# tatsy/opengl-raytracer

Measured on AMD Instinct MI355X. Metric: Mrays/s at 1920x1080, 8 bounces, higher is better.
Workload: dtype f32

## Files before the change

opengl-raytracer_amd/csrc/glrtx.hip:

```cpp
#include "glrtx.h"

#include <hip/hip_runtime.h>

#include <algorithm>
#include <cmath>
#include <cstdarg>
#include <cstdio>
#include <cstdlib>
#include <cstring>
#include <new>
#include <limits>
#include <string>
#include <vector>

#include "glrt_host.h"
#include "pt_kernel.hip.h"
#include "accumulate.hip.h"
#include "lbvh.hip.h"
#include "sahl.hip.h"
#include "refit.hip.h"
#include "skin.hip.h"
#include "normals.hip.h"
#include "query.hip.h"
#include "features.hip.h"
// ... 4253 lines not shown
    nt = std::min(nt, lg.cap_trips);
    std::vector<uint2> tr(nt);
    HIP_TRY(c, hipMemcpy(tr.data(), lg.trips, (size_t)nt * sizeof(uint2), hipMemcpyDeviceToHost));
    unsigned long long logged = 0;
    for (const uint2 &t : tr) logged += t.y;
    DbgLastLaunch L = g_dbg_last;
    L.w.suspend_max = 0;
    using RKernel = void (*)(const KernelArgs, const WfArgs, unsigned *, float4 *, const float4 *, const uint2 *, int);
    int fetch = L.fetch;
    if (const char *v = std::getenv("GLRTX_REPLAY_PAIR_FETCH")) fetch = std::max(0, std::min(2, std::atoi(v)));
    const RKernel rk = fetch == 2 ? (RKernel)pt_replay_traverse<2> : fetch == 1 ? (RKernel)pt_replay_traverse<1> : (RKernel)pt_replay_traverse<0>;
    if (L.lds > 64 * 1024) HIP_TRY(c, hipFuncSetAttribute((const void *)rk, hipFuncAttributeMaxDynamicSharedMemorySize, L.lds));
    int per_cu = 0;
    HIP_TRY(c, hipOccupancyMaxActiveBlocksPerMultiprocessor(&per_cu, rk, kBlockThreads, L.lds));
    if (const char *v = std::getenv("GLRTX_WGS_PER_CU")) per_cu = std::max(1, std::min(per_cu, std::atoi(v)));
    const int grid = std::max(1, std::min(L.grid, per_cu * c->n_cu));
    float ms = 0.f;
    for (int r = 0; r < reps; r++) {
        HIP_TRY(c, hipMemsetAsync(c->work.p, 0, sizeof(unsigned), c->stream));
        HIP_TRY(c, hipEventRecord(c->tm0, c->stream));
        hipLaunchKernelGGL(rk, dim3(grid), dim3(kBlockThreads), L.lds, c->stream, L.a, L.w, (unsigned *)c->work.p, L.queues,
                           (const float4 *)lg.rays, (const uint2 *)lg.trips, (int)nt);
        HIP_TRY(c, hipGetLastError());
        HIP_TRY(c, hipEventRecord(c->tm1, c->stream));
        HIP_TRY(c, hipEventSynchronize(c->tm1));
        HIP_TRY(c, hipEventElapsedTime(&ms, c->tm0, c->tm1));
    }
    out[0] = ms; out[1] = (double)logged; out[2] = (double)nt; out[3] = (double)n;
    return GLRTX_OK;
}
#endif

#ifdef GLRTX_STEP_TIMING
int glrtx_debug_step_timing(unsigned long long out[4]) { return take_symbol(g_step_timing, out); }
#endif

#ifdef GLRTX_PHASE_STATS
int glrtx_debug_trip_log(unsigned out[16 * 64 * 4]) { return take_symbol(g_trip_log, out); }
int glrtx_debug_phase_cycles(unsigned long long out[8]) { return take_symbol(g_phase_cycles, out); }
#endif

int glrtx_timer_begin(glrtx_ctx *c) {
    if (!c) return GLRTX_EINVAL;
    seal_feed(c);
    HIP_TRY(c, hipSetDevice(c->device));
    HIP_TRY(c, hipEventRecord(c->tm0, c->stream));
    return GLRTX_OK;
}

int glrtx_timer_end(glrtx_ctx *c, float *ms) {
    if (!c || !ms) return GLRTX_EINVAL;
    seal_feed(c);
    HIP_TRY(c, hipSetDevice(c->device));
    HIP_TRY(c, hipEventRecord(c->tm1, c->stream));
    HIP_TRY(c, hipEventSynchronize(c->tm1));
    HIP_TRY(c, hipEventElapsedTime(ms, c->tm0, c->tm1));
    return GLRTX_OK;
}

}

struct glrtx_group {
    std::vector<glrtx_ctx *> ctx;
    std::vector<hipEvent_t> done;
    DevBuf full, full8;
    std::vector<char> peer_ok;
    int gather_copies = 0;
// ... 374 lines not shown
```

opengl-raytracer_amd/csrc/pt_kernel.hip.h:

```cpp
#pragma once
#include <hip/hip_runtime.h>
#include <stdint.h>

#include "trav_asm.hip.h"
#include "scan_asm.hip.h"

namespace glrtx {

constexpr int kBlockThreads = 256;
constexpr int kTile = 16;
constexpr int REF_ABSENT = INT32_MIN;
constexpr int REF_FIN = INT32_MIN;
constexpr int kMaxLdsMaterials = 256;
constexpr int kMaxLdsLights = 64;
constexpr int kTopForks = 128;

constexpr float PT_EPS = 1.0e-4f;
constexpr float PT_INFTY = 1.0e8f;
constexpr float PT_PI = 3.14159274101257324f;
constexpr float PT_2PI = 6.28318548202514648f;

struct DevScene {
    const float4 *forks;
    const float4 *nodes0;
// ... 374 lines not shown
        unsigned addr;
        const unsigned lds_base = (unsigned)(uintptr_t)stack;
        asm volatile(
            "s_mov_b64 %[save], exec\n"
            "1:\n\t"
            "v_cmp_ne_u32 vcc, 0, %[sp]\n\t"
            "v_cndmask_b32 %[ref], %[fin], %[ref], vcc\n\t"
            "s_and_b64 exec, exec, vcc\n\t"
            "s_cbranch_execz 2f\n\t"
            "v_add_u32 %[sp], -1, %[sp]\n\t"
            "v_lshl_add_u32 %[addr], %[sp], 11, %[base]\n\t"
            "ds_read_b32 %[ref], %[addr] offset:4\n\t"
            "ds_read_b32 %[t0], %[addr]\n\t"
            "s_waitcnt lgkmcnt(0)\n\t"
            "v_cmp_gt_f32 vcc, %[t0], %[th]\n\t"
            "s_and_b64 exec, exec, vcc\n\t"
            "s_cbranch_execnz 1b\n"
            "2:\n\t"
            "s_mov_b64 exec, %[save]"
            : [t0] "=&v"(t0), [ref] "+&v"(ref), [sp] "+&v"(sp), [save] "=&s"(save), [addr] "=&v"(addr)
            : [base] "v"(lds_base), [th] "v"(T.h.t), [fin] "v"(REF_FIN)
            : "vcc", "scc", "memory");
        static_assert(kBlockThreads * 8 == 1 << 11, "the pop loop shifts the stack index by 11: entry e of lane l at byte (e * kBlockThreads + l) * 8");
        T.sp = sp;
        T.cur = ref;
    }
#ifdef GLRTX_TRAV_STATS
    if (T.cur == REF_FIN) { TS_DONE; }
#endif
    return T.cur == REF_FIN;
}

#ifdef GLRTX_STEP_TIMING
__device__ unsigned long long g_step_timing[4];
struct StepTiming { unsigned t = 0, w = 0, n = 0; };
#define GLRTX_TS_PARAM , StepTiming &ST
#define GLRTX_TS_OPERANDS , [tt] "+&v"(ST.t), [tw] "+&v"(ST.w), [tn] "+&v"(ST.n)
#define GLRTX_TS_CLOBBERS , "s90", "s91", "s92", "s93", "s94", "s95"
#else
#define GLRTX_TS_PARAM
#define GLRTX_TS_OPERANDS
#define GLRTX_TS_CLOBBERS
#endif
constexpr int kWgwfCompact = 8;
constexpr int kWgwfVolume = 16;
template <int FETCH>
DEV void trav_steps_asm(const DevScene &sc, int *stack, Trav &T, unsigned rk GLRTX_TS_PARAM) {
    unsigned long long s_entry, s_act, s_leaf, s_bl, s_br, s_pop, s_tmp;
    const unsigned stk = (unsigned)(uintptr_t)stack;
    static_assert(kBlockThreads * 8 == 1 << 11, "trav_asm.hip.h shifts the stack index by 11: entry e of lane l at byte (e * kBlockThreads + l) * 8");
    static_assert(REF_FIN == INT32_MIN, "trav_asm.hip.h materialises REF_FIN with v_bfrev_b32 v, 1");
    const unsigned par16 = (threadIdx.x & 1u) << 4;
    const unsigned bias_e = sc.node_bias + par16, bias_o = sc.node_bias + 16u - par16;
    if constexpr ((FETCH & kWgwfCompact) != 0) {
        static_assert((FETCH & ~kWgwfCompact) == 0, "the compact layout has the one-record-per-lane fetch only");
        asm volatile(
            "s_mov_b64 %[entry], exec\n\t"
            "s_mov_b64 %[act], exec\n\t"
            GLRTX_ASM_SET_VBASE
            "v_bfrev_b32 v[GLRTX_VB+22], 1\n\t"
            GLRTX_REP(GLRTX_STEPS_PER_TRIP, GLRTX_TRAV_STEP_ASM_COMPACT)
            "99:\n\t"
            "s_mov_b64 exec, %[entry]"
            : [th] "+&v"(T.h.t), [tri] "+&v"(T.h.tri), [hu] "+&v"(T.h.u), [hv] "+&v"(T.h.v), [cur] "+&v"(T.cur), [sp] "+&v"(T.sp),
              [entry] "=&s"(s_entry), [act] "=&s"(s_act), [leaf] "=&s"(s_leaf), [bl] "=&s"(s_bl), [br] "=&s"(s_br), [pop] "=&s"(s_pop), [tmp] "=&s"(s_tmp) GLRTX_TS_OPERANDS
            : [ox] "v"(T.ox), [oy] "v"(T.oy), [oz] "v"(T.oz), [dx] "v"(T.dx), [dy] "v"(T.dy), [dz] "v"(T.dz), [ix] "v"(T.ix), [iy] "v"(T.iy), [iz] "v"(T.iz),
              [sd] "v"(T.stop_d), [stk] "v"(stk), [cbase] "s"(sc.cnodes), [rk] "s"(rk), [eps] "s"(PT_EPS)
            : "vcc", "scc", "memory", GLRTX_ASM_VCLOBBERS_COMPACT GLRTX_TS_CLOBBERS);
        return;
    }
    if (FETCH == 2) {
        asm volatile(
            "s_mov_b64 %[entry], exec\n\t"
            "s_mov_b64 %[act], exec\n\t"
            GLRTX_ASM_SET_VBASE
            "v_bfrev_b32 v[GLRTX_VB+11], 1\n\t"
            GLRTX_REP(GLRTX_STEPS_PER_TRIP_HALF, GLRTX_TRAV_STEP_ASM_PAIR GLRTX_TRAV_STEP_ASM_LANE)
            "99:\n\t"
            "s_mov_b64 exec, %[entry]"
            : [th] "+&v"(T.h.t), [tri] "+&v"(T.h.tri), [hu] "+&v"(T.h.u), [hv] "+&v"(T.h.v), [cur] "+&v"(T.cur), [sp] "+&v"(T.sp),
              [entry] "=&s"(s_entry), [act] "=&s"(s_act), [leaf] "=&s"(s_leaf), [bl] "=&s"(s_bl), [br] "=&s"(s_br), [pop] "=&s"(s_pop), [tmp] "=&s"(s_tmp) GLRTX_TS_OPERANDS
            : [ox] "v"(T.ox), [oy] "v"(T.oy), [oz] "v"(T.oz), [dx] "v"(T.dx), [dy] "v"(T.dy), [dz] "v"(T.dz), [ix] "v"(T.ix), [iy] "v"(T.iy), [iz] "v"(T.iz),
              [sd] "v"(T.stop_d), [stk] "v"(stk), [base] "s"(sc.nodes0), [bias] "s"(sc.node_bias), [eps] "s"(PT_EPS),
              [odd] "s"(0xAAAAAAAAAAAAAAAAull), [biase] "v"(bias_e), [biaso] "v"(bias_o)
            : "vcc", "scc", "memory", GLRTX_ASM_VCLOBBERS_PAIR GLRTX_TS_CLOBBERS);
        return;
    }
    if (FETCH == 1) {
        asm volatile(
            "s_mov_b64 %[entry], exec\n\t"
            "s_mov_b64 %[act], exec\n\t"
            GLRTX_ASM_SET_VBASE
            "v_bfrev_b32 v[GLRTX_VB+11], 1\n\t"
            GLRTX_REP(GLRTX_STEPS_PER_TRIP, GLRTX_TRAV_STEP_ASM_PAIR)
            "99:\n\t"
            "s_mov_b64 exec, %[entry]"
            : [th] "+&v"(T.h.t), [tri] "+&v"(T.h.tri), [hu] "+&v"(T.h.u), [hv] "+&v"(T.h.v), [cur] "+&v"(T.cur), [sp] "+&v"(T.sp),
              [entry] "=&s"(s_entry), [act] "=&s"(s_act), [leaf] "=&s"(s_leaf), [bl] "=&s"(s_bl), [br] "=&s"(s_br), [pop] "=&s"(s_pop), [tmp] "=&s"(s_tmp) GLRTX_TS_OPERANDS
            : [ox] "v"(T.ox), [oy] "v"(T.oy), [oz] "v"(T.oz), [dx] "v"(T.dx), [dy] "v"(T.dy), [dz] "v"(T.dz), [ix] "v"(T.ix), [iy] "v"(T.iy), [iz] "v"(T.iz),
              [sd] "v"(T.stop_d), [stk] "v"(stk), [base] "s"(sc.nodes0), [eps] "s"(PT_EPS),
              [odd] "s"(0xAAAAAAAAAAAAAAAAull), [biase] "v"(bias_e), [biaso] "v"(bias_o)
            : "vcc", "scc", "memory", GLRTX_ASM_VCLOBBERS_PAIR GLRTX_TS_CLOBBERS);
        return;
    }
    asm volatile(
        "s_mov_b64 %[entry], exec\n\t"
        "s_mov_b64 %[act], exec\n\t"
        GLRTX_ASM_SET_VBASE
        "v_bfrev_b32 v[GLRTX_VB+11], 1\n\t"
        GLRTX_REP(GLRTX_STEPS_PER_TRIP, GLRTX_TRAV_STEP_ASM_LANE)
        "99:\n\t"
        "s_mov_b64 exec, %[entry]"
        : [th] "+&v"(T.h.t), [tri] "+&v"(T.h.tri), [hu] "+&v"(T.h.u), [hv] "+&v"(T.h.v), [cur] "+&v"(T.cur), [sp] "+&v"(T.sp),
          [entry] "=&s"(s_entry), [act] "=&s"(s_act), [leaf] "=&s"(s_leaf), [bl] "=&s"(s_bl), [br] "=&s"(s_br), [pop] "=&s"(s_pop), [tmp] "=&s"(s_tmp) GLRTX_TS_OPERANDS
        : [ox] "v"(T.ox), [oy] "v"(T.oy), [oz] "v"(T.oz), [dx] "v"(T.dx), [dy] "v"(T.dy), [dz] "v"(T.dz), [ix] "v"(T.ix), [iy] "v"(T.iy), [iz] "v"(T.iz),
          [sd] "v"(T.stop_d), [stk] "v"(stk), [base] "s"(sc.nodes0), [bias] "s"(sc.node_bias), [eps] "s"(PT_EPS)
        : "vcc", "scc", "memory", GLRTX_ASM_VCLOBBERS GLRTX_TS_CLOBBERS);
}

template <bool CLOSEST>
DEV void tri_test(Hit &h, int t, float ox, float oy, float oz, float dx, float dy, float dz, float v0x, float v0y, float v0z, float e1x,
                  float e1y, float e1z, float e2x, float e2y, float e2z, float tmin = PT_EPS) {
    const float tx = ox - v0x, ty = oy - v0y, tz = oz - v0z;
    const float px = dy * e2z - dz * e2y;
    const float py = dz * e2x - dx * e2z;
    const float pz = dx * e2y - dy * e2x;
    const float det = dot3(e1x, e1y, e1z, px, py, pz);
    const float U = dot3(tx, ty, tz, px, py, pz);
    const float inv = rcp_newton(det);
    const float u = U * inv;
    const bool ok_u = !(-PT_EPS < det && det < PT_EPS) && !(u < 0.0f || 1.0f < u);
    if (!__any(ok_u)) return;
    const float qx = ty * e1z - tz * e1y;
    const float qy = tz * e1x - tx * e1z;
    const float qz = tx * e1y - ty * e1x;
    const float V = dot3(dx, dy, dz, qx, qy, qz);
    const float v = V * inv;
    const bool ok_v = ok_u && !(v < 0.0f || 1.0f < inv * (U + V));
    if (!__any(ok_v)) return;
    const float tt = dot3(e2x, e2y, e2z, qx, qy, qz) * inv;
    const bool hit = ok_v && !(tmin >= tt);
    const bool closer = hit && tt < h.t;
    h.tri = closer ? t : h.tri;
    if (CLOSEST) { h.u = closer ? u : h.u; h.v = closer ? v : h.v; }
// ... 1408 lines not shown
#endif
        if (active) {
#if defined(GLRTX_TRAV_STATS) || defined(GLRTX_CXX_STEP)
            constexpr bool CP = (FETCH & kWgwfCompact) != 0;
            bool fin = trav_step<true, CP>(a.sc, stack, T, ranks);
#pragma unroll
            for (int k = 1; k < GLRTX_STEPS_PER_TRIP; k++)
                if (!fin) fin = trav_step<true, CP>(a.sc, stack, T, ranks);
#else
#ifdef GLRTX_STEP_TIMING
            trav_steps_asm<FETCH>(a.sc, stack, T, (unsigned)(uintptr_t)ranks, step_timing);
#else
            trav_steps_asm<FETCH>(a.sc, stack, T, (unsigned)(uintptr_t)ranks);
#endif
            const bool fin = T.cur == REF_FIN;
#endif
            if (fin) {
                active = false;
                unsaved = true;
            }
        }
#ifdef GLRTX_PHASE_STATS
        ph_step += __builtin_amdgcn_s_memtime() - sb0;
#endif
    }
    if (unsaved) save_hit();
#ifdef GLRTX_PHASE_STATS
    if (threadIdx.x == 0) { atomicAdd(&g_phase_cycles[5], ph_refill); atomicAdd(&g_phase_cycles[6], ph_refills); atomicAdd(&g_phase_cycles[7], ph_step); }
#endif
#ifdef GLRTX_STEP_TIMING
    atomicAdd(&g_step_timing[0], (unsigned long long)step_timing.n);
    atomicAdd(&g_step_timing[1], (unsigned long long)step_timing.t);
    atomicAdd(&g_step_timing[2], (unsigned long long)step_timing.w);
#endif
}

template <bool VOL = false>
DEV void wg_shade_phase(const KernelArgs &a, const WfArgs &w, const float4 *lds_mats, const float *cam, const unsigned *light_bits, int n_paths,
                        float4 *rq_next, unsigned *n_rays_next, unsigned *n_paths_next, unsigned cur_base, unsigned next_base, unsigned long long &rays,
                        unsigned *moved) {
    const int lane = threadIdx.x & 63;
    const unsigned long long lt_mask = (1ull << lane) - 1ull;
    for (int j0 = 0; j0 < n_paths; j0 += kBlockThreads) {
        const int i = j0 + (int)threadIdx.x;
        bool push_ext = false, push_sh = false, requeue = false, has4 = false;
        unsigned id = WF_INVALID;
        float4 ro = make_float4(0.f, 0.f, 0.f, 0.f), rd = ro, rsd = ro, st2 = ro, st3 = ro, st4 = ro;
        const bool light_accepted = i < n_paths && ((light_bits[i >> 5] >> (i & 31)) & 1u) != 0u;
        if (i < n_paths)
            wf_shade_path<VOL>(a, w, lds_mats, cam, id, cur_base + (unsigned)i, light_accepted, push_ext, push_sh, requeue, ro, rd, rsd, st2, st3, st4, has4, rays);
        const unsigned long long me = __ballot(push_ext), ms = __ballot(push_sh), mq = __ballot(requeue), mp = me | ms | mq;
        const unsigned long long mv = __ballot(id != WF_INVALID);
        unsigned br = 0, bp = 0;
        if (lane == 0) {
            if (mv & ~mq) *moved = 1u;
            if (mp) {
                br = atomicAdd(n_rays_next, (unsigned)(__popcll(me) + __popcll(ms)));
                bp = atomicAdd(n_paths_next, (unsigned)__popcll(mp));
            }
        }
        br = __builtin_amdgcn_readfirstlane(br);
        bp = __builtin_amdgcn_readfirstlane(bp);
        const unsigned pos_next = bp + (unsigned)__popcll(mp & lt_mask);
        const unsigned sidx_next = next_base + pos_next;
        if (push_ext || push_sh || requeue) {
            st_stream(w.A(0, sidx_next), ro);
// ... 503 lines not shown
```

opengl-raytracer_amd/csrc/trav_asm.hip.h:

```cpp
#pragma once

#ifndef GLRTX_STEPS_PER_TRIP
#define GLRTX_STEPS_PER_TRIP 6
#endif
#ifndef GLRTX_ASM_VBASE
#define GLRTX_ASM_VBASE 96
#endif
static_assert(GLRTX_STEPS_PER_TRIP % 2 == 0, "the alternating form of the node fetch unrolls steps in pairs");
#define GLRTX_STEPS_PER_TRIP_HALF_(n) GLRTX_HALF_##n
#define GLRTX_HALF_2 1
#define GLRTX_HALF_4 2
#define GLRTX_HALF_6 3
#define GLRTX_HALF_8 4
#define GLRTX_STEPS_PER_TRIP_HALF_X(n) GLRTX_STEPS_PER_TRIP_HALF_(n)
#define GLRTX_STEPS_PER_TRIP_HALF GLRTX_STEPS_PER_TRIP_HALF_X(GLRTX_STEPS_PER_TRIP)
#define GLRTX_STR_(x) #x
#define GLRTX_STR(x) GLRTX_STR_(x)
#define GLRTX_ASM_SET_VBASE ".set GLRTX_VB, " GLRTX_STR(GLRTX_ASM_VBASE) "\n\t"
#if GLRTX_ASM_VBASE == 96
#define GLRTX_ASM_VCLOBBERS "v96", "v97", "v98", "v99", "v100", "v101", "v102", "v103", "v104", "v105", "v106", "v107", "v108", "v109", "v110", "v111", "v112", "v113", "v114", "v115", "v116", "v117"
#define GLRTX_ASM_VCLOBBERS_PAIR GLRTX_ASM_VCLOBBERS, "v118", "v119"
#define GLRTX_ASM_VCLOBBERS_COMPACT GLRTX_ASM_VCLOBBERS_PAIR
#elif GLRTX_ASM_VBASE == 72
#define GLRTX_ASM_VCLOBBERS "v72", "v73", "v74", "v75", "v76", "v77", "v78", "v79", "v80", "v81", "v82", "v83", "v84", "v85", "v86", "v87", "v88", "v89", "v90", "v91", "v92", "v93"
#define GLRTX_ASM_VCLOBBERS_PAIR GLRTX_ASM_VCLOBBERS, "v94", "v95"
#define GLRTX_ASM_VCLOBBERS_COMPACT GLRTX_ASM_VCLOBBERS_PAIR
#else
#error "GLRTX_ASM_VBASE: add the clobber list for this base"
#endif

#ifdef GLRTX_STEP_TIMING
#define GLRTX_TS_BEGIN "s_memtime s[90:91]\n\t"
#define GLRTX_TS_WAIT0 "s_memtime s[92:93]\n\t"
#define GLRTX_TS_WAIT1 "s_memtime s[94:95]\n\ts_waitcnt lgkmcnt(0)\n\ts_sub_u32 s92, s94, s92\n\t"
#define GLRTX_TS_END "s_memtime s[94:95]\n\ts_waitcnt lgkmcnt(0)\n\ts_sub_u32 s94, s94, s90\n\tv_add_u32 %[tt], s94, %[tt]\n\tv_add_u32 %[tw], s92, %[tw]\n\tv_add_u32 %[tn], 1, %[tn]\n\t"
#else
#define GLRTX_TS_BEGIN
#define GLRTX_TS_WAIT0
#define GLRTX_TS_WAIT1
#define GLRTX_TS_END
#endif


#if defined(GLRTX_STEP_TIMING)
#define GLRTX_SINGLE_WAIT
#endif
#ifndef GLRTX_SINGLE_WAIT
#define GLRTX_W3 "s_waitcnt vmcnt(3)\n\t"
#define GLRTX_W2 "s_waitcnt vmcnt(2)\n\t"
#define GLRTX_W1 "s_waitcnt vmcnt(1)\n\t"
#define GLRTX_W0 "s_waitcnt vmcnt(0)\n\t"
#else
#define GLRTX_W3 "s_waitcnt vmcnt(0)\n\t"
#define GLRTX_W2
#define GLRTX_W1
#define GLRTX_W0
#endif
#define GLRTX_TRAV_STEP_ASM_PAIR \
    GLRTX_TS_BEGIN \
    "s_andn2_b64 %[tmp], %[act], %[odd]\n\t"    \
    "s_lshl_b64 %[tmp], %[tmp], 1\n\t" \
    "s_and_b64 %[pop], %[act], %[odd]\n\t" \
    "s_lshr_b64 %[pop], %[pop], 1\n\t" \
    "s_or_b64 %[tmp], %[tmp], %[pop]\n\t" \
    "s_or_b64 %[pop], %[tmp], %[act]\n\t"    \
    "s_mov_b64 exec, %[pop]\n\t" \
    "v_cndmask_b32_e64 v[GLRTX_VB+4], -1, %[cur], %[act]\n\t"    \
    "v_cmp_gt_i32_e64 %[leaf], 0, %[cur]\n\t"    \
    "s_nop 0\n\t"    \
    "v_mov_b32_dpp v[GLRTX_VB+15], v[GLRTX_VB+4] quad_perm:[0,0,2,2] row_mask:0xf bank_mask:0xf\n\t"    \
    "v_mov_b32_dpp v[GLRTX_VB+23], v[GLRTX_VB+4] quad_perm:[1,1,3,3] row_mask:0xf bank_mask:0xf\n\t"    \
    "v_lshl_add_u32 v[GLRTX_VB+15], v[GLRTX_VB+15], 6, %[biase]\n\t"    \
// ... 176 lines not shown
    "v_max_f32 v[GLRTX_VB+17], v[GLRTX_VB+5], v[GLRTX_VB+1]\n\t" \
    "v_min_f32 v[GLRTX_VB+1], v[GLRTX_VB+5], v[GLRTX_VB+1]\n\t" \
    "v_max_f32 v[GLRTX_VB+18], v[GLRTX_VB+6], v[GLRTX_VB+2]\n\t" \
    "v_min_f32 v[GLRTX_VB+4], v[GLRTX_VB+6], v[GLRTX_VB+2]\n\t" \
    "v_min3_f32 v[GLRTX_VB+16], v[GLRTX_VB+16], v[GLRTX_VB+17], v[GLRTX_VB+18]\n\t"    \
    "v_max3_f32 v[GLRTX_VB+2], v[GLRTX_VB+0], v[GLRTX_VB+1], v[GLRTX_VB+4]\n\t"        \
    "v_min_f32 v[GLRTX_VB+16], v[GLRTX_VB+16], %[th]\n\t" \
    "v_cmp_ge_f32_e64 %[bl], v[GLRTX_VB+16], v[GLRTX_VB+2]\n\t"                      \
    GLRTX_CW0 \
    "v_sub_f32 v[GLRTX_VB+8], v[GLRTX_VB+8], %[ox]\n\t"    \
    "v_sub_f32 v[GLRTX_VB+9], v[GLRTX_VB+9], %[oy]\n\t" \
    "v_sub_f32 v[GLRTX_VB+10], v[GLRTX_VB+10], %[oz]\n\t" \
    "v_mul_f32 v[GLRTX_VB+8], v[GLRTX_VB+8], %[ix]\n\t" \
    "v_mul_f32 v[GLRTX_VB+9], v[GLRTX_VB+9], %[iy]\n\t" \
    "v_mul_f32 v[GLRTX_VB+10], v[GLRTX_VB+10], %[iz]\n\t" \
    "v_sub_f32 v[GLRTX_VB+12], v[GLRTX_VB+3], %[ox]\n\t" \
    "v_sub_f32 v[GLRTX_VB+13], v[GLRTX_VB+7], %[oy]\n\t" \
    "v_sub_f32 v[GLRTX_VB+14], v[GLRTX_VB+11], %[oz]\n\t" \
    "v_mul_f32 v[GLRTX_VB+12], v[GLRTX_VB+12], %[ix]\n\t" \
    "v_mul_f32 v[GLRTX_VB+13], v[GLRTX_VB+13], %[iy]\n\t" \
    "v_mul_f32 v[GLRTX_VB+14], v[GLRTX_VB+14], %[iz]\n\t" \
    "v_max_f32 v[GLRTX_VB+16], v[GLRTX_VB+12], v[GLRTX_VB+8]\n\t" \
    "v_min_f32 v[GLRTX_VB+8], v[GLRTX_VB+12], v[GLRTX_VB+8]\n\t" \
    "v_max_f32 v[GLRTX_VB+17], v[GLRTX_VB+13], v[GLRTX_VB+9]\n\t" \
    "v_min_f32 v[GLRTX_VB+9], v[GLRTX_VB+13], v[GLRTX_VB+9]\n\t" \
    "v_max_f32 v[GLRTX_VB+18], v[GLRTX_VB+14], v[GLRTX_VB+10]\n\t" \
    "v_min_f32 v[GLRTX_VB+10], v[GLRTX_VB+14], v[GLRTX_VB+10]\n\t" \
    "v_min3_f32 v[GLRTX_VB+16], v[GLRTX_VB+16], v[GLRTX_VB+17], v[GLRTX_VB+18]\n\t" \
    "v_max3_f32 v[GLRTX_VB+8], v[GLRTX_VB+8], v[GLRTX_VB+9], v[GLRTX_VB+10]\n\t" \
    "v_min_f32 v[GLRTX_VB+16], v[GLRTX_VB+16], %[th]\n\t" \
    "v_cmp_ge_f32_e64 %[br], v[GLRTX_VB+16], v[GLRTX_VB+8]\n\t" \
    "v_lshl_add_u32 v[GLRTX_VB+3], v[GLRTX_VB+19], 1, 1\n\t"                         \
    "v_add_u32 v[GLRTX_VB+7], 1, v[GLRTX_VB+3]\n\t"                                  \
    GLRTX_TRAV_STEP_TAIL_X("", "v[GLRTX_VB+22]")
#define GLRTX_TRAV_STEP_TAIL GLRTX_TRAV_STEP_TAIL_X("v_not_b32 v[GLRTX_VB+3], %[cur]\n\t", "v[GLRTX_VB+11]")
#define GLRTX_TRAV_STEP_TAIL_X(TRI, FIN) \
    "v_cndmask_b32_e64 %[cur], v[GLRTX_VB+3], v[GLRTX_VB+7], %[br]\n\t"                                  \
    "s_or_b64 %[tmp], %[bl], %[br]\n\t"                                                                                                                \
    "s_andn2_b64 %[pop], exec, %[tmp]\n\t"                                                                     \
    "s_and_b64 exec, %[bl], %[br]\n\t"                                                               \
    "v_lshl_add_u32 v[GLRTX_VB+15], %[sp], 11, %[stk]\n\t"                                                                                                       \
    "ds_write_b64 v[GLRTX_VB+15], v[GLRTX_VB+2:GLRTX_VB+3]\n\t"                                                                                                                  \
    "v_add_u32 %[sp], 1, %[sp]\n\t"                                                                                                                    \
    "s_and_b64 exec, %[act], %[leaf]\n\t"                                \
    "s_cbranch_scc0 21f\n\t"                                                                                                                           \
    TRI                                                                                                                                      \
    "v_mov_b32 %[cur], v[GLRTX_VB+7]\n\t"                                                   \
    "v_mul_f32 v[GLRTX_VB+16], %[dy], v[GLRTX_VB+10]\n\t"                                                                                                  \
    "v_mul_f32 v[GLRTX_VB+19], %[dz], v[GLRTX_VB+9]\n\t"                                                                                                                  \
    "v_sub_f32 v[GLRTX_VB+16], v[GLRTX_VB+16], v[GLRTX_VB+19]\n\t"                                                                                                                   \
    "v_mul_f32 v[GLRTX_VB+17], %[dz], v[GLRTX_VB+8]\n\t"                                                                                                                  \
    "v_mul_f32 v[GLRTX_VB+19], %[dx], v[GLRTX_VB+10]\n\t"                                                                                                                  \
    "v_sub_f32 v[GLRTX_VB+17], v[GLRTX_VB+17], v[GLRTX_VB+19]\n\t"                                                                                                                   \
    "v_mul_f32 v[GLRTX_VB+18], %[dx], v[GLRTX_VB+9]\n\t"                                                                                                                  \
    "v_mul_f32 v[GLRTX_VB+19], %[dy], v[GLRTX_VB+8]\n\t"                                                                                                                  \
    "v_sub_f32 v[GLRTX_VB+18], v[GLRTX_VB+18], v[GLRTX_VB+19]\n\t"                                                                                                                   \
    "v_mul_f32 v[GLRTX_VB+20], v[GLRTX_VB+6], v[GLRTX_VB+18]\n\t"                                                                          \
    "v_mul_f32 v[GLRTX_VB+19], v[GLRTX_VB+5], v[GLRTX_VB+17]\n\t"                                                                                                                   \
    "v_add_f32 v[GLRTX_VB+20], v[GLRTX_VB+20], v[GLRTX_VB+19]\n\t"                                                                                                                   \
    "v_mul_f32 v[GLRTX_VB+19], v[GLRTX_VB+4], v[GLRTX_VB+16]\n\t"                                                                                                                   \
    "v_add_f32 v[GLRTX_VB+20], v[GLRTX_VB+20], v[GLRTX_VB+19]\n\t"                                                                                                                   \
    "v_rcp_f32 v[GLRTX_VB+21], v[GLRTX_VB+20]\n\t"                                                                                                                         \
    "v_sub_f32 v[GLRTX_VB+0], %[ox], v[GLRTX_VB+0]\n\t"                                                                                          \
    "v_sub_f32 v[GLRTX_VB+1], %[oy], v[GLRTX_VB+1]\n\t"                                                                                                                    \
    "v_sub_f32 v[GLRTX_VB+2], %[oz], v[GLRTX_VB+2]\n\t"                                                                                                                    \
    "v_fma_f32 v[GLRTX_VB+19], -v[GLRTX_VB+20], v[GLRTX_VB+21], 1.0\n\t"                                                           \
    "v_fma_f32 v[GLRTX_VB+21], v[GLRTX_VB+19], v[GLRTX_VB+21], v[GLRTX_VB+21]\n\t"                                                                                                             \
    "v_mul_f32 v[GLRTX_VB+18], v[GLRTX_VB+2], v[GLRTX_VB+18]\n\t"                                                                                   \
    "v_mul_f32 v[GLRTX_VB+19], v[GLRTX_VB+1], v[GLRTX_VB+17]\n\t"                                                                                                                    \
    "v_add_f32 v[GLRTX_VB+18], v[GLRTX_VB+18], v[GLRTX_VB+19]\n\t"                                                                                                                   \
    "v_mul_f32 v[GLRTX_VB+19], v[GLRTX_VB+0], v[GLRTX_VB+16]\n\t"                                                                                                                    \
    "v_add_f32 v[GLRTX_VB+18], v[GLRTX_VB+18], v[GLRTX_VB+19]\n\t"                                                                                                                   \
    "v_mul_f32 v[GLRTX_VB+15], v[GLRTX_VB+18], v[GLRTX_VB+21]\n\t"                                                                                                            \
    "v_cmpx_nlt_f32_e64 %[tmp], |v[GLRTX_VB+20]|, %[eps]\n\t"                                                                    \
    "v_cmpx_ngt_f32 vcc, 0, v[GLRTX_VB+15]\n\t"                                                                                                    \
// ... 10 lines not shown
    "v_sub_f32 v[GLRTX_VB+14], v[GLRTX_VB+14], v[GLRTX_VB+19]\n\t"                                                                                                                   \
    "v_mul_f32 v[GLRTX_VB+7], %[dz], v[GLRTX_VB+14]\n\t"                                                                                 \
    "v_mul_f32 v[GLRTX_VB+19], %[dy], v[GLRTX_VB+13]\n\t"                                                                                                                  \
    "v_add_f32 v[GLRTX_VB+7], v[GLRTX_VB+7], v[GLRTX_VB+19]\n\t"                                                                                                                   \
    "v_mul_f32 v[GLRTX_VB+19], %[dx], v[GLRTX_VB+12]\n\t"                                                                                                                  \
    "v_add_f32 v[GLRTX_VB+7], v[GLRTX_VB+7], v[GLRTX_VB+19]\n\t"                                                                                                                   \
    "v_mul_f32 v[GLRTX_VB+16], v[GLRTX_VB+7], v[GLRTX_VB+21]\n\t"                                                                                                            \
    "v_add_f32 v[GLRTX_VB+19], v[GLRTX_VB+18], v[GLRTX_VB+7]\n\t"                                                                                                                   \
    "v_mul_f32 v[GLRTX_VB+19], v[GLRTX_VB+21], v[GLRTX_VB+19]\n\t"                                                                       \
    "v_cmpx_ngt_f32 vcc, 0, v[GLRTX_VB+16]\n\t"                                                                                                    \
    "v_cmpx_nlt_f32 vcc, 1.0, v[GLRTX_VB+19]\n\t"                                                                                        \
    "s_cbranch_execz 20f\n\t"                                                                                                                          \
    "v_mul_f32 v[GLRTX_VB+19], v[GLRTX_VB+10], v[GLRTX_VB+14]\n\t"                                                                      \
    "v_mul_f32 v[GLRTX_VB+7], v[GLRTX_VB+9], v[GLRTX_VB+13]\n\t"                                                                                                                   \
    "v_add_f32 v[GLRTX_VB+19], v[GLRTX_VB+19], v[GLRTX_VB+7]\n\t"                                                                                                                   \
    "v_mul_f32 v[GLRTX_VB+7], v[GLRTX_VB+8], v[GLRTX_VB+12]\n\t"                                                                                                                   \
    "v_add_f32 v[GLRTX_VB+19], v[GLRTX_VB+19], v[GLRTX_VB+7]\n\t"                                                                                                                   \
    "v_mul_f32 v[GLRTX_VB+19], v[GLRTX_VB+19], v[GLRTX_VB+21]\n\t"                                                                                                                   \
    "v_cmpx_nge_f32 vcc, %[eps], v[GLRTX_VB+19]\n\t"                                                                                            \
    "v_cmpx_lt_f32 vcc, v[GLRTX_VB+19], %[th]\n\t"                                                 \
    "v_mov_b32 %[tri], v[GLRTX_VB+3]\n\t"                                                                                                                        \
    "v_mov_b32 %[hu], v[GLRTX_VB+15]\n\t"                                                                                                                        \
    "v_mov_b32 %[hv], v[GLRTX_VB+16]\n\t"                                                                                                                        \
    "v_mov_b32 %[th], v[GLRTX_VB+19]\n\t"                                                                                                                        \
    "20:\n\t"                                                                                                                                          \
    "s_and_b64 exec, %[act], %[leaf]\n\t"                                                                                   \
    "v_sub_f32 v[GLRTX_VB+16], %[sd], %[th]\n\t"                                                            \
    "v_cmp_nle_f32 vcc, %[eps], v[GLRTX_VB+16]\n\t"                                                               \
    "v_cndmask_b32 %[cur], " FIN ", %[cur], vcc\n\t"                       \
    "v_cmp_eq_u32_e64 %[tmp], %[cur], " FIN "\n\t"                                                                                                       \
    "s_and_b64 vcc, vcc, %[tmp]\n\t"                                                            \
    "s_or_b64 %[pop], %[pop], vcc\n\t"                                                                                                                \
    "21:\n\t"                                                                                                                                          \
    "s_mov_b64 exec, %[pop]\n\t"                                         \
    "s_cbranch_execz 30f\n\t"                                                                                                                          \
    "10:\n\t"                                                                                                                                          \
    "v_cmp_ne_u32 vcc, 0, %[sp]\n\t"                                                                                                                   \
    "v_cndmask_b32 %[cur], " FIN ", %[cur], vcc\n\t"                                                                \
    "s_and_b64 exec, exec, vcc\n\t"                                                                                                                    \
    "s_cbranch_execz 30f\n\t"                                                                                                                          \
    "v_add_u32 %[sp], -1, %[sp]\n\t"                                                                                                                   \
    "v_lshl_add_u32 v[GLRTX_VB+15], %[sp], 11, %[stk]\n\t"                                                                                                       \
    "ds_read_b64 v[GLRTX_VB+16:GLRTX_VB+17], v[GLRTX_VB+15]\n\t"                                                                                                  \
    "s_waitcnt lgkmcnt(0)\n\t"                                                                                                                         \
    "v_mov_b32 %[cur], v[GLRTX_VB+17]\n\t"                                                                                                                       \
    "v_cmp_gt_f32 vcc, v[GLRTX_VB+16], %[th]\n\t"                                                                                                                \
    "s_and_b64 exec, exec, vcc\n\t"                                                                                                                    \
    "s_cbranch_execnz 10b\n\t"                                                                                                                         \
    "30:\n\t"                                                                                                                                          \
    "s_mov_b64 exec, %[act]\n\t"                                                                                  \
    GLRTX_TS_END                                                                                                                       \
    "v_cmpx_ne_u32_e64 %[act], %[cur], " FIN "\n\t"                                                                             \
    "s_cbranch_execz 99f\n\t"

#define GLRTX_REP1(X) X
#define GLRTX_REP2(X) X X
#define GLRTX_REP3(X) X X X
#define GLRTX_REP4(X) X X X X
#define GLRTX_REP5(X) X X X X X
#define GLRTX_REP6(X) X X X X X X
#define GLRTX_REP7(X) X X X X X X X
#define GLRTX_REP8(X) X X X X X X X X
#define GLRTX_REP_(N, X) GLRTX_REP##N(X)
#define GLRTX_REP(N, X) GLRTX_REP_(N, X)
```

Baseline: 10340.

## Cache stack top in registers and prefetch next LDS entry during traversal pops

```diff
diff --git a/opengl-raytracer_amd/csrc/glrtx.hip b/opengl-raytracer_amd/csrc/glrtx.hip
--- a/opengl-raytracer_amd/csrc/glrtx.hip
+++ b/opengl-raytracer_amd/csrc/glrtx.hip
@@ -4309,7 +4309,7 @@
 #endif
 
 #ifdef GLRTX_STEP_TIMING
-int glrtx_debug_step_timing(unsigned long long out[4]) { return take_symbol(g_step_timing, out); }
+int glrtx_debug_step_timing(unsigned long long out[8]) { return take_symbol(g_step_timing, out); }
 #endif
 
 #ifdef GLRTX_PHASE_STATS
diff --git a/opengl-raytracer_amd/csrc/pt_kernel.hip.h b/opengl-raytracer_amd/csrc/pt_kernel.hip.h
--- a/opengl-raytracer_amd/csrc/pt_kernel.hip.h
+++ b/opengl-raytracer_amd/csrc/pt_kernel.hip.h
@@ -430,11 +430,11 @@
 }
 
 #ifdef GLRTX_STEP_TIMING
-__device__ unsigned long long g_step_timing[4];
-struct StepTiming { unsigned t = 0, w = 0, n = 0; };
+__device__ unsigned long long g_step_timing[8];
+struct StepTiming { unsigned t = 0, w = 0, n = 0, p = 0, q = 0, i = 0, c = 0; };
 #define GLRTX_TS_PARAM , StepTiming &ST
-#define GLRTX_TS_OPERANDS , [tt] "+&v"(ST.t), [tw] "+&v"(ST.w), [tn] "+&v"(ST.n)
-#define GLRTX_TS_CLOBBERS , "s90", "s91", "s92", "s93", "s94", "s95"
+#define GLRTX_TS_OPERANDS , [tt] "+&v"(ST.t), [tw] "+&v"(ST.w), [tn] "+&v"(ST.n), [tp] "+&v"(ST.p), [tq] "+&v"(ST.q), [ti] "+&v"(ST.i), [tc] "+&v"(ST.c)
+#define GLRTX_TS_CLOBBERS , "s82", "s83", "s84", "s85", "s86", "s87", "s88", "s89", "s90", "s91", "s92", "s93", "s94", "s95"
 #else
 #define GLRTX_TS_PARAM
 #define GLRTX_TS_OPERANDS
@@ -457,8 +457,10 @@
             "s_mov_b64 %[act], exec\n\t"
             GLRTX_ASM_SET_VBASE
             "v_bfrev_b32 v[GLRTX_VB+22], 1\n\t"
+            GLRTX_TOP_ENTER
             GLRTX_REP(GLRTX_STEPS_PER_TRIP, GLRTX_TRAV_STEP_ASM_COMPACT)
             "99:\n\t"
+            GLRTX_TOP_LANDED
             "s_mov_b64 exec, %[entry]"
             : [th] "+&v"(T.h.t), [tri] "+&v"(T.h.tri), [hu] "+&v"(T.h.u), [hv] "+&v"(T.h.v), [cur] "+&v"(T.cur), [sp] "+&v"(T.sp),
               [entry] "=&s"(s_entry), [act] "=&s"(s_act), [leaf] "=&s"(s_leaf), [bl] "=&s"(s_bl), [br] "=&s"(s_br), [pop] "=&s"(s_pop), [tmp] "=&s"(s_tmp) GLRTX_TS_OPERANDS
@@ -473,8 +475,10 @@
             "s_mov_b64 %[act], exec\n\t"
             GLRTX_ASM_SET_VBASE
             "v_bfrev_b32 v[GLRTX_VB+11], 1\n\t"
+            GLRTX_TOP_ENTER
             GLRTX_REP(GLRTX_STEPS_PER_TRIP_HALF, GLRTX_TRAV_STEP_ASM_PAIR GLRTX_TRAV_STEP_ASM_LANE)
             "99:\n\t"
+            GLRTX_TOP_LANDED
             "s_mov_b64 exec, %[entry]"
             : [th] "+&v"(T.h.t), [tri] "+&v"(T.h.tri), [hu] "+&v"(T.h.u), [hv] "+&v"(T.h.v), [cur] "+&v"(T.cur), [sp] "+&v"(T.sp),
               [entry] "=&s"(s_entry), [act] "=&s"(s_act), [leaf] "=&s"(s_leaf), [bl] "=&s"(s_bl), [br] "=&s"(s_br), [pop] "=&s"(s_pop), [tmp] "=&s"(s_tmp) GLRTX_TS_OPERANDS
@@ -490,8 +494,10 @@
             "s_mov_b64 %[act], exec\n\t"
             GLRTX_ASM_SET_VBASE
             "v_bfrev_b32 v[GLRTX_VB+11], 1\n\t"
+            GLRTX_TOP_ENTER
             GLRTX_REP(GLRTX_STEPS_PER_TRIP, GLRTX_TRAV_STEP_ASM_PAIR)
             "99:\n\t"
+            GLRTX_TOP_LANDED
             "s_mov_b64 exec, %[entry]"
             : [th] "+&v"(T.h.t), [tri] "+&v"(T.h.tri), [hu] "+&v"(T.h.u), [hv] "+&v"(T.h.v), [cur] "+&v"(T.cur), [sp] "+&v"(T.sp),
               [entry] "=&s"(s_entry), [act] "=&s"(s_act), [leaf] "=&s"(s_leaf), [bl] "=&s"(s_bl), [br] "=&s"(s_br), [pop] "=&s"(s_pop), [tmp] "=&s"(s_tmp) GLRTX_TS_OPERANDS
@@ -506,8 +512,10 @@
         "s_mov_b64 %[act], exec\n\t"
         GLRTX_ASM_SET_VBASE
         "v_bfrev_b32 v[GLRTX_VB+11], 1\n\t"
+        GLRTX_TOP_ENTER
         GLRTX_REP(GLRTX_STEPS_PER_TRIP, GLRTX_TRAV_STEP_ASM_LANE)
         "99:\n\t"
+        GLRTX_TOP_LANDED
         "s_mov_b64 exec, %[entry]"
         : [th] "+&v"(T.h.t), [tri] "+&v"(T.h.tri), [hu] "+&v"(T.h.u), [hv] "+&v"(T.h.v), [cur] "+&v"(T.cur), [sp] "+&v"(T.sp),
           [entry] "=&s"(s_entry), [act] "=&s"(s_act), [leaf] "=&s"(s_leaf), [bl] "=&s"(s_bl), [br] "=&s"(s_br), [pop] "=&s"(s_pop), [tmp] "=&s"(s_tmp) GLRTX_TS_OPERANDS
@@ -1982,6 +1990,10 @@
     atomicAdd(&g_step_timing[0], (unsigned long long)step_timing.n);
     atomicAdd(&g_step_timing[1], (unsigned long long)step_timing.t);
     atomicAdd(&g_step_timing[2], (unsigned long long)step_timing.w);
+    atomicAdd(&g_step_timing[3], (unsigned long long)step_timing.p);
+    atomicAdd(&g_step_timing[4], (unsigned long long)step_timing.q);
+    atomicAdd(&g_step_timing[5], (unsigned long long)step_timing.i);
+    atomicAdd(&g_step_timing[6], (unsigned long long)step_timing.c);
 #endif
 }
 
diff --git a/opengl-raytracer_amd/csrc/trav_asm.hip.h b/opengl-raytracer_amd/csrc/trav_asm.hip.h
--- a/opengl-raytracer_amd/csrc/trav_asm.hip.h
+++ b/opengl-raytracer_amd/csrc/trav_asm.hip.h
@@ -18,11 +18,11 @@
 #define GLRTX_STR(x) GLRTX_STR_(x)
 #define GLRTX_ASM_SET_VBASE ".set GLRTX_VB, " GLRTX_STR(GLRTX_ASM_VBASE) "\n\t"
 #if GLRTX_ASM_VBASE == 96
-#define GLRTX_ASM_VCLOBBERS "v96", "v97", "v98", "v99", "v100", "v101", "v102", "v103", "v104", "v105", "v106", "v107", "v108", "v109", "v110", "v111", "v112", "v113", "v114", "v115", "v116", "v117"
+#define GLRTX_ASM_VCLOBBERS "v96", "v97", "v98", "v99", "v100", "v101", "v102", "v103", "v104", "v105", "v106", "v107", "v108", "v109", "v110", "v111", "v112", "v113", "v114", "v115", "v116", "v117", "v94", "v95"
 #define GLRTX_ASM_VCLOBBERS_PAIR GLRTX_ASM_VCLOBBERS, "v118", "v119"
 #define GLRTX_ASM_VCLOBBERS_COMPACT GLRTX_ASM_VCLOBBERS_PAIR
 #elif GLRTX_ASM_VBASE == 72
-#define GLRTX_ASM_VCLOBBERS "v72", "v73", "v74", "v75", "v76", "v77", "v78", "v79", "v80", "v81", "v82", "v83", "v84", "v85", "v86", "v87", "v88", "v89", "v90", "v91", "v92", "v93"
+#define GLRTX_ASM_VCLOBBERS "v72", "v73", "v74", "v75", "v76", "v77", "v78", "v79", "v80", "v81", "v82", "v83", "v84", "v85", "v86", "v87", "v88", "v89", "v90", "v91", "v92", "v93", "v70", "v71"
 #define GLRTX_ASM_VCLOBBERS_PAIR GLRTX_ASM_VCLOBBERS, "v94", "v95"
 #define GLRTX_ASM_VCLOBBERS_COMPACT GLRTX_ASM_VCLOBBERS_PAIR
 #else
@@ -33,11 +33,21 @@
 #define GLRTX_TS_BEGIN "s_memtime s[90:91]\n\t"
 #define GLRTX_TS_WAIT0 "s_memtime s[92:93]\n\t"
 #define GLRTX_TS_WAIT1 "s_memtime s[94:95]\n\ts_waitcnt lgkmcnt(0)\n\ts_sub_u32 s92, s94, s92\n\t"
-#define GLRTX_TS_END "s_memtime s[94:95]\n\ts_waitcnt lgkmcnt(0)\n\ts_sub_u32 s94, s94, s90\n\tv_add_u32 %[tt], s94, %[tt]\n\tv_add_u32 %[tw], s92, %[tw]\n\tv_add_u32 %[tn], 1, %[tn]\n\t"
+#define GLRTX_TS_POP0 "s_memtime s[84:85]\n\ts_mov_b32 s82, 0\n\ts_mov_b32 s83, 0\n\t"
+#define GLRTX_TS_POPIT "s_add_u32 s83, s83, 1\n\t"
+#define GLRTX_TS_POPW0 "s_memtime s[86:87]\n\t"
+#define GLRTX_TS_POPW1 "s_memtime s[88:89]\n\ts_waitcnt lgkmcnt(0)\n\ts_sub_u32 s86, s88, s86\n\ts_add_u32 s82, s82, s86\n\t"
+#define GLRTX_TS_END "s_memtime s[94:95]\n\ts_waitcnt lgkmcnt(0)\n\ts_memtime s[88:89]\n\ts_waitcnt lgkmcnt(0)\n\ts_sub_u32 s88, s88, s94\n\ts_sub_u32 s84, s94, s84\n\ts_sub_u32 s94, s94, s90\n\t" \
+    "v_add_u32 %[tt], s94, %[tt]\n\tv_add_u32 %[tw], s92, %[tw]\n\tv_add_u32 %[tn], 1, %[tn]\n\t" \
+    "v_add_u32 %[tp], s84, %[tp]\n\tv_add_u32 %[tq], s82, %[tq]\n\tv_add_u32 %[ti], s83, %[ti]\n\tv_add_u32 %[tc], s88, %[tc]\n\t"
 #else
 #define GLRTX_TS_BEGIN
 #define GLRTX_TS_WAIT0
 #define GLRTX_TS_WAIT1
+#define GLRTX_TS_POP0
+#define GLRTX_TS_POPIT
+#define GLRTX_TS_POPW0
+#define GLRTX_TS_POPW1
 #define GLRTX_TS_END
 #endif
 
@@ -280,15 +290,70 @@
     "v_cmp_ge_f32_e64 %[br], v[GLRTX_VB+16], v[GLRTX_VB+8]\n\t" \
     "v_lshl_add_u32 v[GLRTX_VB+3], v[GLRTX_VB+19], 1, 1\n\t"                         \
     "v_add_u32 v[GLRTX_VB+7], 1, v[GLRTX_VB+3]\n\t"                                  \
-    GLRTX_TRAV_STEP_TAIL_X("", "v[GLRTX_VB+22]")
-#define GLRTX_TRAV_STEP_TAIL GLRTX_TRAV_STEP_TAIL_X("v_not_b32 v[GLRTX_VB+3], %[cur]\n\t", "v[GLRTX_VB+11]")
-#define GLRTX_TRAV_STEP_TAIL_X(TRI, FIN) \
+    GLRTX_TRAV_STEP_TAIL_X("", "v[GLRTX_VB+22]", "")
+#ifndef GLRTX_POP_WAIT
+#define GLRTX_TOP_ENTER \
+    "v_cmp_ne_u32 vcc, 0, %[sp]\n\t"                                               \
+    "s_and_b64 exec, exec, vcc\n\t" \
+    "v_add_u32 v[GLRTX_VB+15], -1, %[sp]\n\t" \
+    "v_lshl_add_u32 v[GLRTX_VB+15], v[GLRTX_VB+15], 11, %[stk]\n\t" \
+    "ds_read_b64 v[GLRTX_VB-2:GLRTX_VB-1], v[GLRTX_VB+15]\n\t"                        \
+    "s_mov_b64 exec, %[act]\n\t"
+#define GLRTX_TOP_LANDED "s_waitcnt lgkmcnt(0)\n\t"
+#define GLRTX_TOP_PUSH "v_mov_b64 v[GLRTX_VB-2:GLRTX_VB-1], v[GLRTX_VB+2:GLRTX_VB+3]\n\t"
+#define GLRTX_TRAV_POP_EMPTY(FIN) \
+    "v_cmp_ne_u32 vcc, 0, %[sp]\n\t"                                                                                                                   \
+    "v_cndmask_b32 %[cur], " FIN ", %[cur], vcc\n\t"                                                                \
+    "s_and_b64 exec, exec, vcc\n\t"                                                                                                                    \
+    "s_cbranch_execz 30f\n\t"
+#define GLRTX_TRAV_POP_TAKE \
+    GLRTX_TS_POPIT                                                                                                                     \
+    "v_mov_b32 %[cur], v[GLRTX_VB-1]\n\t"                                                                                                             \
+    "v_cmp_gt_f32 vcc, v[GLRTX_VB-2], %[th]\n\t"                                                                                                      \
+    "v_sub_u32_e64 v[GLRTX_VB+15], %[sp], 2 clamp\n\t"                         \
+    "v_add_u32 %[sp], -1, %[sp]\n\t"                                                                                                                   \
+    "v_lshl_add_u32 v[GLRTX_VB+15], v[GLRTX_VB+15], 11, %[stk]\n\t"                                                                                    \
+    "ds_read_b64 v[GLRTX_VB-2:GLRTX_VB-1], v[GLRTX_VB+15]\n\t"                                              \
+    "s_and_b64 exec, exec, vcc\n\t"
+#define GLRTX_TRAV_POP(FIN) \
+    GLRTX_TRAV_POP_EMPTY(FIN)                                                                                                          \
+    GLRTX_TRAV_POP_TAKE                                                                                                                \
+    "s_cbranch_execz 30f\n\t"                                                                                                                          \
+    "10:\n\t"                                                                                               \
+    GLRTX_TRAV_POP_EMPTY(FIN)                                                                                                          \
+    GLRTX_TS_POPW0 "s_waitcnt lgkmcnt(0)\n\t" GLRTX_TS_POPW1                                                                           \
+    GLRTX_TRAV_POP_TAKE                                                                                                                \
+    "s_cbranch_execnz 10b\n\t"
+#else
+#define GLRTX_TOP_ENTER
+#define GLRTX_TOP_LANDED
+#define GLRTX_TOP_PUSH
+#define GLRTX_TRAV_POP(FIN) \
+    "10:\n\t"                                                                                                                                          \
+    "v_cmp_ne_u32 vcc, 0, %[sp]\n\t"                                                                                                                   \
+    "v_cndmask_b32 %[cur], " FIN ", %[cur], vcc\n\t"                                                                \
+    "s_and_b64 exec, exec, vcc\n\t"                                                                                                                    \
+    "s_cbranch_execz 30f\n\t"                                                                                                                          \
+    GLRTX_TS_POPIT                                                                                                                     \
+    "v_add_u32 %[sp], -1, %[sp]\n\t"                                                                                                                   \
+    "v_lshl_add_u32 v[GLRTX_VB+15], %[sp], 11, %[stk]\n\t"                                                                                                       \
+    "ds_read_b64 v[GLRTX_VB+16:GLRTX_VB+17], v[GLRTX_VB+15]\n\t"                                                                                                  \
+    GLRTX_TS_POPW0 "s_waitcnt lgkmcnt(0)\n\t" GLRTX_TS_POPW1                                                                           \
+    "v_mov_b32 %[cur], v[GLRTX_VB+17]\n\t"                                                                                                                       \
+    "v_cmp_gt_f32 vcc, v[GLRTX_VB+16], %[th]\n\t"                                                                                                                \
+    "s_and_b64 exec, exec, vcc\n\t"                                                                                                                    \
+    "s_cbranch_execnz 10b\n\t"
+#endif
+#define GLRTX_TRAV_STEP_TAIL GLRTX_TRAV_STEP_TAIL_X("v_not_b32 v[GLRTX_VB+3], %[cur]\n\t", "v[GLRTX_VB+11]", GLRTX_TOP_LANDED)
+#define GLRTX_TRAV_STEP_TAIL_X(TRI, FIN, LANDED) \
     "v_cndmask_b32_e64 %[cur], v[GLRTX_VB+3], v[GLRTX_VB+7], %[br]\n\t"                                  \
     "s_or_b64 %[tmp], %[bl], %[br]\n\t"                                                                                                                \
     "s_andn2_b64 %[pop], exec, %[tmp]\n\t"                                                                     \
     "s_and_b64 exec, %[bl], %[br]\n\t"                                                               \
+    LANDED                                                                         \
     "v_lshl_add_u32 v[GLRTX_VB+15], %[sp], 11, %[stk]\n\t"                                                                                                       \
     "ds_write_b64 v[GLRTX_VB+15], v[GLRTX_VB+2:GLRTX_VB+3]\n\t"                                                                                                                  \
+    GLRTX_TOP_PUSH                                                                                                      \
     "v_add_u32 %[sp], 1, %[sp]\n\t"                                                                                                                    \
     "s_and_b64 exec, %[act], %[leaf]\n\t"                                \
     "s_cbranch_scc0 21f\n\t"                                                                                                                           \
@@ -365,21 +430,10 @@
     "s_and_b64 vcc, vcc, %[tmp]\n\t"                                                            \
     "s_or_b64 %[pop], %[pop], vcc\n\t"                                                                                                                \
     "21:\n\t"                                                                                                                                          \
+    GLRTX_TS_POP0                                                                                                                      \
     "s_mov_b64 exec, %[pop]\n\t"                                         \
     "s_cbranch_execz 30f\n\t"                                                                                                                          \
-    "10:\n\t"                                                                                                                                          \
-    "v_cmp_ne_u32 vcc, 0, %[sp]\n\t"                                                                                                                   \
-    "v_cndmask_b32 %[cur], " FIN ", %[cur], vcc\n\t"                                                                \
-    "s_and_b64 exec, exec, vcc\n\t"                                                                                                                    \
-    "s_cbranch_execz 30f\n\t"                                                                                                                          \
-    "v_add_u32 %[sp], -1, %[sp]\n\t"                                                                                                                   \
-    "v_lshl_add_u32 v[GLRTX_VB+15], %[sp], 11, %[stk]\n\t"                                                                                                       \
-    "ds_read_b64 v[GLRTX_VB+16:GLRTX_VB+17], v[GLRTX_VB+15]\n\t"                                                                                                  \
-    "s_waitcnt lgkmcnt(0)\n\t"                                                                                                                         \
-    "v_mov_b32 %[cur], v[GLRTX_VB+17]\n\t"                                                                                                                       \
-    "v_cmp_gt_f32 vcc, v[GLRTX_VB+16], %[th]\n\t"                                                                                                                \
-    "s_and_b64 exec, exec, vcc\n\t"                                                                                                                    \
-    "s_cbranch_execnz 10b\n\t"                                                                                                                         \
+    GLRTX_TRAV_POP(FIN)                                                                                                                \
     "30:\n\t"                                                                                                                                          \
     "s_mov_b64 exec, %[act]\n\t"                                                                                  \
     GLRTX_TS_END                                                                                                                       \
```

After: 10410 (median of 6 runs). No clear change (+0.8%).
